# arobertlin/MinPaxos

Measured on AMD Instinct MI355X. Metric: decided+applied instances/sec (tally + KV apply + RCCL watermark all-reduce), higher is better.
Workload: dtype int32/int64

## Files before the change

### minpaxos_amd/csrc/step.hip

```cpp
#include "common.hpp"
#include "kernels.hpp"
#include "tally.hpp"

namespace mpx {

#ifndef MPX_STAMPS
#define MPX_STAMPS 0
#endif
#if MPX_STAMPS
__device__ unsigned long long mpx_stamp_acc[16];
constexpr uint32_t kSpanMax = 1u << 17;
__device__ unsigned long long mpx_wg_span[kSpanMax][2];
#define STAMP_DECL                                                     \
    unsigned long long _st_prev = 0, _st_rt0 = 0;                      \
    if (threadIdx.x == 0) {                                            \
        _st_prev = __builtin_amdgcn_s_memtime();                       \
        _st_rt0 = __builtin_amdgcn_s_memrealtime();                    \
    }
#define STAMP_SPAN()                                                   \
    do {                                                               \
        if (MPX_STAMPS >= 2 && threadIdx.x == 0 && blockIdx.x < kSpanMax) { \
            mpx_wg_span[blockIdx.x][0] = _st_rt0;                      \
            mpx_wg_span[blockIdx.x][1] = __builtin_amdgcn_s_memrealtime(); \
        }                                                              \
    } while (0)
#define STAMP(k)                                                       \
    do {                                                               \
        if (MPX_STAMPS == 1 && threadIdx.x == 0) {  \
            unsigned long long _n = __builtin_amdgcn_s_memtime();      \
            atomicAdd(&mpx_stamp_acc[k], _n - _st_prev);               \
            _st_prev = _n;                                             \
        }                                                              \
    } while (0)
#else
#define STAMP_DECL
#define STAMP(k)
#define STAMP_SPAN()
#endif
#ifndef MPX_ABLATE
#define MPX_ABLATE 0
#endif

#ifndef MPX_STEP_BALLOT
#define MPX_STEP_BALLOT 0
#endif

constexpr int kStepBlock = 256;
constexpr uint32_t kLock = 0xFFFFFFFFu;
constexpr uint32_t kDead = 0xFFFFFFFEu;
constexpr uint32_t kNoFirst = 0xFFFFFFFFu;

__device__ __forceinline__ uint32_t lhash(int64_t k) {
    uint64_t x = (uint64_t)k;
    x ^= x >> 33;
    x *= 0xff51afd7ed558ccdull;
    x ^= x >> 33;
    return (uint32_t)x;
}

struct Dict {
    int64_t* dkey;
    int64_t* dval;
    uint32_t* dfirst;
    uint32_t* cnt;
    uint32_t* hslot;
    uint8_t* dpresent;
    uint8_t* dseen;
    uint32_t* dn;
    uint32_t dcap, hcap;
};

__device__ int dict_insert(const Dict& D, int64_t key) {
    uint32_t h = lhash(key) & (D.hcap - 1);
    for (uint32_t probe = 0; probe < D.hcap;) {
        uint32_t cur = __hip_atomic_load(&D.hslot[h], __ATOMIC_ACQUIRE, __HIP_MEMORY_SCOPE_WORKGROUP);
        if (cur == 0) {
            const uint32_t old = atomicCAS(&D.hslot[h], 0u, kLock);
            if (old == 0) {
                const uint32_t kid = atomicAdd(D.dn, 1u);
                if (kid >= D.dcap) {
                    __hip_atomic_store(&D.hslot[h], kDead, __ATOMIC_RELEASE, __HIP_MEMORY_SCOPE_WORKGROUP);
                    return -1;
                }
                D.dkey[kid] = key;
                D.dval[kid] = 0;
                D.dpresent[kid] = 0;
                D.dseen[kid] = 0;
                D.dfirst[kid] = kNoFirst;
                D.cnt[kid] = 0;
                __hip_atomic_store(&D.hslot[h], kid + 1, __ATOMIC_RELEASE, __HIP_MEMORY_SCOPE_WORKGROUP);
                return (int)kid;
            }
            cur = old;
        }
        if (cur == kLock) continue;
        if (cur != kDead && D.dkey[cur - 1] == key) return (int)(cur - 1);
        h = (h + 1) & (D.hcap - 1);
        ++probe;
    }
    return -1;
}

__device__ __forceinline__ void dict_put_unique(const Dict& D, uint32_t e, int64_t k, int64_t v) {
    D.dkey[e] = k;
    D.dval[e] = v;
    D.dpresent[e] = 1;
    D.dseen[e] = 0;
    D.dfirst[e] = kNoFirst;
    uint32_t h = lhash(k) & (D.hcap - 1);
    while (atomicCAS(&D.hslot[h], 0u, e + 1) != 0u) h = (h + 1) & (D.hcap - 1);
}

template <int PER, typename OffT>
__device__ __forceinline__ void block_scan(const uint32_t* cnt, OffT* off, uint32_t n,
                                           uint32_t* wsum) {
    const int t = threadIdx.x, l = lane_id(), w = t / kWave;
    uint32_t v[PER];
    uint32_t sum = 0;
#pragma unroll
    for (int k = 0; k < PER; ++k) {
        const uint32_t i = t * PER + k;
        v[k] = i < n ? cnt[i] : 0;
        sum += v[k];
    }
    uint32_t incl = sum;
#pragma unroll
    for (int d = 1; d < kWave; d <<= 1) {
        const uint32_t x = __shfl_up(incl, d);
        if (l >= d) incl += x;
    }
    if (l == kWave - 1) wsum[w] = incl;
    __syncthreads();
    uint32_t wbase = 0;
    for (int k = 0; k < w; ++k) wbase += wsum[k];
    uint32_t run = wbase + incl - sum;
#pragma unroll
    for (int k = 0; k < PER; ++k) {
        const uint32_t i = t * PER + k;
        if (i < n) off[i] = (OffT)run;
        run += v[k];
    }
    __syncthreads();
}

template <typename OffT>
__device__ __forceinline__ uint8_t resolve_cmd(const Dict& D, const OffT* off,
                                               const uint16_t* list, const int64_t* cval, int kd,
                                               uint32_t li, uint8_t o, int64_t& r, bool& conf) {
    const bool isput = o == MPX_OP_PUT;
    int prev = -1, prevput = 0, lastput = -1;
    bool later = false, laterput = false;
    const uint32_t a = off[kd], z = a + D.cnt[kd];
    for (uint32_t j = a; j < z; ++j) {
        const uint32_t ent = list[j];
        const int lj = (int)(ent >> 1);
        const uint32_t pj = ent & 1u;
        if (lj < (int)li) {
            if (lj > prev) { prev = lj; prevput = (int)pj; }
            if (pj && lj > lastput) lastput = lj;
        } else if (lj > (int)li) {
            later = true;
            laterput |= pj != 0;
        }
    }
    const uint8_t seen = D.dseen[kd];
    if (prev >= 0) conf = prevput || isput;
    else conf = (seen & 1u) && ((seen & 2u) || isput);
    r = 0;
    if (isput) r = cval[li];
    else if (o == MPX_OP_GET) {
        if (lastput >= 0) r = cval[lastput];
        else if (D.dpresent[kd]) r = D.dval[kd];
    }
    uint8_t fl = 0;
    if (!later) fl |= 1;
    if (isput && !laterput) fl |= 2;
    if (isput && lastput < 0) fl |= 4;
    return fl;
}

__device__ __forceinline__ void apply_update(const Dict& D, int kd, uint8_t fl, uint8_t o,
                                             int64_t v, uint32_t first_pos, uint32_t n_orig) {
    if (fl & 1) D.dseen[kd] = (uint8_t)(1u | (o == MPX_OP_PUT ? 2u : 0u));
    if (fl & 2) {
        D.dval[kd] = v;
        D.dpresent[kd] = 1;
    }
    if ((fl & 4) && (uint32_t)kd >= n_orig && D.dfirst[kd] == kNoFirst) D.dfirst[kd] = first_pos;
}

__device__ __forceinline__ void table_writeback(const Dict& D, uint32_t norig, uint32_t dn,
                                                int64_t* kk, int64_t* kv, uint32_t kvpg,
                                                uint32_t* total, uint32_t* err) {
    const int t = threadIdx.x;
    for (uint32_t e = t; e < norig; e += kStepBlock) {
        kk[e] = D.dkey[e];
        kv[e] = D.dval[e];
    }
    if (t == 0) *total = norig;
    __syncthreads();
    for (uint32_t e = norig + t; e < dn; e += kStepBlock) {
        if (!D.dpresent[e]) continue;
        const uint32_t f = D.dfirst[e];
        uint32_t rank = 0;
        for (uint32_t x = norig; x < dn; ++x)
            if (D.dpresent[x] && D.dfirst[x] < f) ++rank;
        atomicAdd(total, 1u);
        const uint32_t dst = norig + rank;
        if (dst < kvpg) {
            kk[dst] = D.dkey[e];
            kv[dst] = D.dval[e];
        }
    }
    __syncthreads();
    if (t == 0 && *total > kvpg) raise_err(err, kErrKvFull);
}

template <int T_, int R_, int C_, int TB_, int HB_, int HN_ = (1 << HB_)>
struct FastCfg {
    static constexpr int kFT = T_, kFRecs = R_, kFIpg = T_, kFCmds = C_, kFTab = TB_;
    static constexpr int kFHB = HB_, kFH = HN_;
    static constexpr bool kFHPow2 = (HN_ & (HN_ - 1)) == 0;
    static_assert(HN_ <= (1 << HB_) && HN_ >= TB_ && HN_ % 8 == 0, "slot count");
    static constexpr int kFPer = kFCmds / kFT;
    static constexpr int kFRecPer = kFRecs / kFT;
    static constexpr int kFTabPer = (kFTab + kFT - 1) / kFT;
    static constexpr int kFWaves = kFT / kWave;
    static constexpr int kWaveCmds = kFCmds / kFWaves;
#ifndef MPX_DVAL_LDS_MAX
#define MPX_DVAL_LDS_MAX 512
#endif
    static constexpr bool kFDvalLds = TB_ <= MPX_DVAL_LDS_MAX;
    static_assert(kFCmds % kFT == 0 && kFRecs % kFT == 0, "whole items per thread");
    static_assert(kFCmds / 32 <= kWave, "the new-key bitmap is scanned by one wave");
    static_assert(kWaveCmds < 2047, "kTabLp holds 1 + a wave-relative command index");
    static_assert((kFH * 2) % 16 == 0, "the wave tables are cleared by 16-byte stores");
};
#ifndef MPX_FASTBASE_SLOTS
#define MPX_FASTBASE_SLOTS 512
#endif
using FastBase = FastCfg<256, 1024, 1024, 256, 9, MPX_FASTBASE_SLOTS>;
using FastRecs = FastCfg<256, 2048, 1024, 256, 9>;
using FastKeys = FastCfg<256, 1024, 1024, 1024, 10>;
using FastWide = FastCfg<512, 2048, 2048, 512, 10>;
using FastWide256 = FastCfg<512, 2048, 2048, 256, 9>;
constexpr uint16_t kNone16 = 0xFFFF;
constexpr uint8_t kIdBad = 31;
constexpr unsigned long long kFreeKey = 0x8000000000000000ull;
constexpr uint32_t kOverflow = 0x80000000u;
constexpr uint32_t kTabAny = 0x8000u;
constexpr uint32_t kTabPut = 0x4000u;
constexpr uint32_t kTabLp = 0x07FFu;

#define MPX_FAST_CONSTS                                                      \
    constexpr int kFT = Cfg::kFT, kFRecs = Cfg::kFRecs, kFIpg = Cfg::kFIpg;    \
    constexpr int kFCmds = Cfg::kFCmds, kFTab = Cfg::kFTab, kFH = Cfg::kFH;    \
    constexpr int kFPer = Cfg::kFPer, kFRecPer = Cfg::kFRecPer;                \
    constexpr int kFTabPer = Cfg::kFTabPer, kFWaves = Cfg::kFWaves;            \
    constexpr int kWaveCmds = Cfg::kWaveCmds;                                   \
    (void)kFT; (void)kFRecs; (void)kFIpg; (void)kFCmds; (void)kFTab; (void)kFH; \
    (void)kFPer; (void)kFRecPer; (void)kFTabPer; (void)kFWaves; (void)kWaveCmds;

template <class Cfg, int MODE>
struct FastLds {
    static constexpr int kFRecs = Cfg::kFRecs, kFIpg = Cfg::kFIpg, kFCmds = Cfg::kFCmds;
    static constexpr int kFTab = Cfg::kFTab, kFH = Cfg::kFH, kFWaves = Cfg::kFWaves;
    union {
        struct {
            int32_t inst[kFRecs];
            int32_t bal[MODE == MPX_MODE_CLASSIC ? kFRecs : 1];
            uint8_t idok[kFRecs];
            uint16_t rstart[kFIpg];
            uint16_t rend[kFIpg];
        } a;
        struct {
            int64_t cval[kFCmds];
            uint16_t tab[kFWaves * kFH];
#if !MPX_STEP_BALLOT
            uint8_t win[kFWaves * kFH];
            unsigned long long pmask[kFWaves * kWave];
#endif
        } b;
    } u;
    unsigned long long hkey[kFH];
    int64_t dval[Cfg::kFDvalLds ? kFTab : 1];
    uint16_t tabidx[kFH];
    uint32_t newbits[kFCmds / 32];
    uint16_t coff[kFIpg + 2];
    uint32_t red[1 + MPX_MAX_REPLICAS];
    uint32_t firstnil, firstbad, flags, ndec;
#ifdef MPX_LDS_PAD
    uint8_t lds_pad[MPX_LDS_PAD];
#endif
};

__device__ __forceinline__ uint32_t wave_max_u32(uint32_t v) {
#pragma unroll
    for (int d = 32; d >= 1; d >>= 1) {
        const uint32_t x = __shfl_xor(v, d);
        v = v > x ? v : x;
    }
    return (uint32_t)__builtin_amdgcn_readfirstlane((int)v);
}

template <int HB>
__device__ __forceinline__ uint32_t fhash(int64_t k) {
    const uint32_t x = (uint32_t)(uint64_t)k ^ (uint32_t)((uint64_t)k >> 32);
    return (x * 0x9E3779B1u) >> (32 - HB);
}
template <class Cfg>
__device__ __forceinline__ uint32_t fhome(int64_t k) {
    if constexpr (Cfg::kFHPow2) {
        return fhash<Cfg::kFHB>(k);
    } else {
        const uint32_t x = (uint32_t)(uint64_t)k ^ (uint32_t)((uint64_t)k >> 32);
        return (uint32_t)(((uint64_t)(x * 0x9E3779B1u) * (uint32_t)Cfg::kFH) >> 32);
    }
}

template <class Cfg, class Lds>
__device__ __forceinline__ int fast_slot(Lds& S, unsigned long long key, uint32_t h,
                                         int& fresh) {
    constexpr int kFH = Cfg::kFH;
    uint32_t i = h;
    for (int probe = 0; probe < kFH; ++probe) {
        const unsigned long long old = atomicCAS(&S.hkey[i], kFreeKey, key);
        if (old == kFreeKey || old == key) {
            fresh = old == kFreeKey;
            return (int)i;
        }
        i = Cfg::kFHPow2 ? (i + 1) & (kFH - 1) : (i + 1 == (uint32_t)kFH ? 0u : i + 1);
    }
    return -1;
}

constexpr uint32_t kPkGroups = 64;
__device__ __forceinline__ unsigned long long pk_word(uint32_t d, uint32_t xi, uint32_t xc) {
    return 1ull | ((unsigned long long)d << 7) | ((unsigned long long)xi << 23) |
           ((unsigned long long)xc << 39);
}
__device__ __forceinline__ uint32_t pk_slots(uint32_t n_groups) {
    return (n_groups + kPkGroups - 1) / kPkGroups;
}
__device__ void fold_packed(unsigned long long* pslots, uint32_t n_groups, int64_t* totals,
                            uint32_t* err) {
    __shared__ unsigned long long fsum[3];
    if (threadIdx.x < 3) fsum[threadIdx.x] = 0;
    __syncthreads();
    unsigned long long d = 0, xi = 0, xc = 0;
    const uint32_t nslots = pk_slots(n_groups);
    constexpr int kBatch = 2;
    for (uint32_t s0 = threadIdx.x; s0 < nslots; s0 += blockDim.x * kBatch) {
        unsigned long long w[kBatch];
#pragma unroll
        for (int k = 0; k < kBatch; ++k) {
            const uint32_t sl = s0 + k * blockDim.x;
            w[k] = sl < nslots ? __hip_atomic_load(pslots + sl, __ATOMIC_RELAXED,
                                                   __HIP_MEMORY_SCOPE_AGENT)
                               : 0ull;
        }
#pragma unroll
        for (int k = 0; k < kBatch; ++k) {
            const uint32_t sl = s0 + k * blockDim.x;
            if (sl >= nslots) continue;
            const uint32_t want = (n_groups - 1u - sl) / nslots + 1u;
            uint32_t spins = 0;
            bool late = false;
            while ((w[k] & 127ull) < want) {
                __builtin_amdgcn_s_sleep(2);
                w[k] = __hip_atomic_load(pslots + sl, __ATOMIC_RELAXED, __HIP_MEMORY_SCOPE_AGENT);
                if (++spins == (1u << 22)) {
                    raise_err(err, kErrInval | kErrSlots);
                    late = true;
                    break;
                }
            }
            if (!late) __hip_atomic_store(pslots + sl, 0ull, __ATOMIC_RELAXED, __HIP_MEMORY_SCOPE_AGENT);
            d += (w[k] >> 7) & 0xFFFFull;
            xi += (w[k] >> 23) & 0xFFFFull;
            xc += w[k] >> 39;
        }
    }
    if (d) atomicAdd(&fsum[0], d);
    if (xi) atomicAdd(&fsum[1], xi);
    if (xc) atomicAdd(&fsum[2], xc);
    __syncthreads();
    if (threadIdx.x < 3) totals[threadIdx.x] = (int64_t)fsum[threadIdx.x];
}

template <int MODE, class Cfg, bool kOne>
__global__ __launch_bounds__(Cfg::kFT) void k_group_fast(mpx_group_batch b, int32_t nrep,
                                                         uint32_t kvpg, uint32_t* worklist,
                                                         uint32_t* wcount,
                                                         unsigned long long* tacc, uint32_t* err,
                                                         unsigned long long* pslots,
                                                         int64_t* totals) {
    if constexpr (!kOne) {
        pslots = nullptr;
        totals = nullptr;
    }
    MPX_FAST_CONSTS
    __shared__ FastLds<Cfg, MODE> S;
    STAMP_DECL
    const uint32_t g = blockIdx.x;
    const int t = threadIdx.x, l = lane_id();
    const int32_t half = nrep >> 1;
    const uint32_t ipg = b.ipg;
    const uint64_t gi0 = (uint64_t)g * ipg;
    const uint64_t r0 = b.grp_rec_off[g], r1 = b.grp_rec_off[g + 1];
    const uint32_t c_lo = b.cmd_off[gi0], c_hi = b.cmd_off[gi0 + ipg];
    const uint32_t kcnt = b.kv_cnt_in[g];
    const int32_t cu_in = b.committed_in[g];
    const int32_t ex_in = b.executed_in[g];
    const uint64_t nrec = r1 - r0;
    const uint32_t ncmd = c_hi - c_lo;
    if (r1 < r0 || c_hi < c_lo || nrec > (uint64_t)kFRecs || ncmd > (uint32_t)kFCmds ||
        kcnt > (uint32_t)kFTab || kcnt > kvpg) {
        if (pslots) {
            if (t == 0) {
                raise_err(err, kErrInval);
                if (totals) (void)__hip_atomic_fetch_add(pslots + g % pk_slots(gridDim.x), 1ull, __ATOMIC_RELAXED,
                                                         __HIP_MEMORY_SCOPE_AGENT);
            }
            if (totals && g == gridDim.x - 1) fold_packed(pslots, gridDim.x, totals, err);
        } else if (t == 0) {
            worklist[atomicAdd(wcount, 1u)] = g;
        }
        return;
    }
    const int64_t lo = (int64_t)ex_in + 1 < 0 ? 0 : (int64_t)ex_in + 1;
    uint32_t ebits = 0;

    int4 rr[kFRecPer];
    if (nrec) {
        const uint32_t last = (uint32_t)nrec - 1;
#pragma unroll
        for (int k = 0; k < kFRecPer; ++k) {
            const uint32_t p = t + k * kFT;
            rr[k] = ld_stream(reinterpret_cast<const int4*>(b.recs) + r0 + (p < last ? p : last));
        }
    } else {
#pragma unroll
        for (int k = 0; k < kFRecPer; ++k) rr[k] = make_int4(-1, 0, 0, 0);
    }
    const bool own = (uint32_t)t < ipg;
    const uint32_t ti = own ? (uint32_t)t : ipg - 1;
    int4 st = ld_stream(reinterpret_cast<const int4*>(b.st_in) + gi0 + ti);
    const uint32_t co = b.cmd_off[gi0 + ti];
    const uint8_t hs = b.has_cmds ? b.has_cmds[gi0 + ti] : (uint8_t)1;
    int64_t tk[kFTabPer], tv[kFTabPer];
#pragma unroll
    for (int k = 0; k < kFTabPer; ++k) {
        const uint32_t e = (uint32_t)t + k * kFT;
        const uint64_t ei = (uint64_t)g * kvpg + (e < kcnt ? e : (kcnt ? kcnt - 1 : 0));
        tk[k] = b.kv_key_in[ei];
        tv[k] = b.kv_val_in[ei];
    }
#pragma unroll
    for (int k = 0; k < (kFH + kFT - 1) / kFT; ++k)
        if (kFH % kFT == 0 || t + k * kFT < kFH) S.hkey[t + k * kFT] = kFreeKey;
    for (int i = t; i < kFH / 2; i += kFT)
        reinterpret_cast<uint32_t*>(S.tabidx)[i] = 0xFFFFFFFFu;
    if (t < kFCmds / 32) S.newbits[t] = 0u;
    S.u.a.rstart[t] = kNone16;
    S.coff[t] = (uint16_t)(own ? co - c_lo : ncmd);
    if (t <= MPX_MAX_REPLICAS) S.red[t] = 0;
    if (t == 0) {
        S.coff[kFIpg] = (uint16_t)ncmd;
        S.firstnil = ipg;
        S.firstbad = ipg;
        S.flags = 0;
        S.ndec = 0;
    }
#pragma unroll
    for (int k = 0; k < kFRecPer; ++k) {
        const uint32_t p = t + k * kFT;
        const uint32_t idc = (rr[k].z >= 0 && rr[k].z < nrep) ? (uint32_t)rr[k].z : kIdBad;
        S.u.a.inst[p] = rr[k].x;
        if (MODE == MPX_MODE_CLASSIC) S.u.a.bal[p] = rr[k].y;
        S.u.a.idok[p] = (uint8_t)((idc << 1) | ((rr[k].w & 0xff) == 1 ? 1u : 0u));
    }
    const uint32_t clast = ncmd ? ncmd - 1 : 0;
    const uint32_t cbase = (uint32_t)(t - l) * kFPer + (uint32_t)l;
    uint8_t o[kFPer];
    int64_t ck[kFPer];
#pragma unroll
    for (int k = 0; k < kFPer; ++k) {
        const uint32_t li = cbase + k * kWave;
        const uint64_t ci = c_lo + (li < clast ? li : clast);
        o[k] = ncmd ? ld_stream(b.op + ci) : (uint8_t)0;
        ck[k] = ncmd ? ld_stream(b.key + ci) : 0;
    }
    __syncthreads();
    STAMP(0);

#pragma unroll
    for (int k = 0; k < kFRecPer; ++k) {
        const uint32_t p = t + k * kFT;
        const bool valid = p < nrec;
        const int32_t inst = S.u.a.inst[p];
        const int32_t prev = S.u.a.inst[p ? p - 1 : 0];
        const bool inwin = inst >= 0 && (uint32_t)inst < ipg;
        const bool pinwin = prev >= 0 && (uint32_t)prev < ipg;
        const bool head = valid && (p == 0 || inst != prev);
        ebits |= (valid && !inwin) ? kErrNil : 0u;
        ebits |= (head && p && inst < prev) ? kErrOrder : 0u;
        if (head && inwin) S.u.a.rstart[inst] = (uint16_t)p;
        if (head && p && pinwin) S.u.a.rend[prev] = (uint16_t)p;
        if (valid && p + 1 == nrec && inwin) S.u.a.rend[inst] = (uint16_t)nrec;
    }
    int tslot[kFTabPer];
#pragma unroll
    for (int k = 0; k < kFTabPer; ++k) {
        const uint32_t e = (uint32_t)t + k * kFT;
        tslot[k] = 0;
        if (e < kcnt) {
            int fresh = 0;
            const int sl = (unsigned long long)tk[k] == kFreeKey
                               ? -1
                               : fast_slot<Cfg>(S, (unsigned long long)tk[k], fhome<Cfg>(tk[k]),
                                           fresh);
            ebits |= sl < 0 ? kOverflow : 0u;
            tslot[k] = sl < 0 ? 0 : sl;
            if (fresh) S.tabidx[sl] = (uint16_t)e;
            if (Cfg::kFDvalLds) S.dval[e] = tv[k];
        }
    }
    __syncthreads();
    STAMP(1);

    bool dec = false;
#if MPX_ABLATE & 8
    const uint32_t ra = (uint32_t)t * 4;
    const bool touched = true;
    const uint32_t rn = 4;
#else
    const uint32_t ra = own ? S.u.a.rstart[t] : kNone16;
    const bool touched = ra != kNone16;
    const uint32_t rn = touched ? (uint32_t)S.u.a.rend[t] - ra : 0;
#endif
#if MPX_ABLATE & 1
    const uint32_t rmax = 0;
#else
    const uint32_t rmax = wave_max_u32(rn);
#endif
    if (MODE == MPX_MODE_MIN) {
        uint32_t idmask = 0;
        int32_t deci = 0;
        for (uint32_t j = 0; j < rmax; ++j) {
            const uint32_t p = j < rn ? ra + j : 0;
            const uint32_t io0 = S.u.a.idok[p];
            const uint32_t io = j < rn ? io0 : 0u;
            const int32_t okj = (int32_t)(io & 1u);
            const uint32_t nilbit = st.x == MPX_STATUS_NIL ? kErrNil : 0u;
            ebits |= okj ? nilbit : 0u;
            const int32_t oks = st.y + okj;
            const int32_t c1 = oks >= half ? okj : 0;
            const int32_t dj = oks == half ? c1 : 0;
            st.y = oks;
            st.x = dj ? MPX_COMMITTED : st.x;
            deci |= dj;
            const uint32_t id = io >> 1;
            const uint32_t badbit = id == kIdBad ? kErrBadId : 0u;
            ebits |= c1 ? badbit : 0u;
            idmask |= c1 ? (1u << id) : 0u;
        }
        dec = deci != 0;
        const uint32_t wbase = (uint32_t)(t - l) + 1;
        const unsigned long long dm = __ballot(deci != 0);
        if (l == 0 && dm) atomicMax(&S.red[0], wbase + 63u - (uint32_t)__clzll(dm));
        for (int i = 0; i < nrep; ++i) {
            const unsigned long long m = __ballot((idmask >> i) & 1u);
            if (l == 0 && m) atomicMax(&S.red[1 + i], wbase + 63u - (uint32_t)__clzll(m));
        }
    } else {
        ebits |= (touched && st.x == MPX_STATUS_NIL) ? kErrNil : 0u;
        int32_t deci = 0;
        for (uint32_t j = 0; j < rmax; ++j) {
            const uint32_t p = j < rn ? ra + j : 0;
            const int32_t act = j < rn ? 1 : 0;
            const int32_t io = (int32_t)S.u.a.idok[p];
            const int32_t bj = S.u.a.bal[p];
            const int32_t live = (uint32_t)(st.x - MPX_PREPARED) < 2u ? act : 0;
            const int32_t okj = live & io & 1;
            const int32_t nk = live & ((io & 1) ^ 1);
            const int32_t oks = st.y + okj;
            const int32_t c = oks >= half ? okj : 0;
            st.y = oks;
            st.x = c ? MPX_COMMITTED : st.x;
            deci |= c;
            st.z += nk;
            const int32_t nb = nk ? bj : INT32_MIN;
            st.w = st.w > nb ? st.w : nb;
        }
        dec = deci != 0;
        if (__ballot(dec) && l == 0) atomicMax(&S.red[0], 1u);
    }
    {
        const unsigned long long dm = __ballot(dec);
        if (l == 0 && dm) atomicAdd(&S.ndec, (uint32_t)__popcll(dm));
    }
    {
        uint32_t fn = (own && (int64_t)t >= lo && (st.x == MPX_STATUS_NIL || !hs)) ? (uint32_t)t : ipg;
        uint32_t fb = (MODE == MPX_MODE_CLASSIC && own && (int64_t)t >= (int64_t)cu_in + 1 &&
                       st.x != MPX_COMMITTED) ? (uint32_t)t : ipg;
#pragma unroll
        for (int d = 32; d >= 1; d >>= 1) {
            const uint32_t x = __shfl_xor(fn, d), y = __shfl_xor(fb, d);
            fn = fn < x ? fn : x;
            fb = fb < y ? fb : y;
        }
        if (l == 0) {
            if (fn < ipg) atomicMin(&S.firstnil, fn);
            if (MODE == MPX_MODE_CLASSIC && fb < ipg) atomicMin(&S.firstbad, fb);
        }
    }
    __syncthreads();
    STAMP(2);

    int32_t cu = cu_in;
    if (MPX_ABLATE & 32) {
        cu = (int32_t)ipg - 1;
    } else if (MODE == MPX_MODE_MIN) {
        if (S.red[0]) cu = (int32_t)S.red[0] - 1;
    } else if (S.red[0] && (int64_t)cu_in + 1 >= 0 && (int64_t)cu_in + 1 < (int64_t)ipg) {
        cu = (int32_t)S.firstbad - 1;
    }
    int64_t hi = (int64_t)cu;
    if (hi >= (int64_t)ipg) hi = (int64_t)ipg - 1;
    int64_t stop = hi >= lo ? hi + 1 : lo;
    if ((int64_t)S.firstnil < stop && (int64_t)S.firstnil >= lo) stop = S.firstnil;
    const uint32_t x0 = stop > lo ? S.coff[lo] : 0, x1 = stop > lo ? S.coff[stop] : 0;

    int64_t cv[kFPer];
#pragma unroll
    for (int k = 0; k < kFPer; ++k) {
        const uint32_t li = cbase + k * kWave;
        cv[k] = ncmd ? ld_stream(b.val + c_lo + (li < clast ? li : clast)) : 0;
    }
    uint32_t ops = 0;
#pragma unroll
    for (int k = 0; k < kFPer; ++k) ops |= (uint32_t)o[k] << (8 * k);
    const int wv = __builtin_amdgcn_readfirstlane(t / kWave);
    uint16_t* T = S.u.b.tab + wv * kFH;
#pragma unroll
    for (int k = 0; k < (kFH * 2 / 16 + kWave - 1) / kWave; ++k)
        if ((kFH * 2 / 16) % kWave == 0 || l + k * kWave < kFH * 2 / 16)
            reinterpret_cast<uint4*>(T)[l + k * kWave] = make_uint4(0u, 0u, 0u, 0u);
#if !MPX_STEP_BALLOT
    typedef __attribute__((address_space(3))) volatile uint8_t lds_u8;
    typedef __attribute__((address_space(3))) volatile unsigned long long lds_u64;
    lds_u8* W = (lds_u8*)(S.u.b.win + wv * kFH);
    lds_u64* PM = (lds_u64*)(S.u.b.pmask + wv * kWave);
    PM[l] = 0ull;
#endif
    const unsigned long long lanebit = 1ull << l;
    const unsigned long long below = lanebit - 1ull;
    const uint32_t wfirst = (uint32_t)wv * kWaveCmds;
    int kid[kFPer];
    uint32_t seen[kFPer];
#pragma unroll
    for (int k = 0; k < kFPer; ++k) {
        const uint32_t li = cbase + k * kWave;
        const bool act = li >= x0 && li < x1;
        const unsigned long long key = (unsigned long long)ck[k];
        int kd = -1;
#if MPX_ABLATE & 2
        if (act) kd = (int)fhome<Cfg>(ck[k]);
#else
        if (act && key != kFreeKey) {
            int fresh = 0;
            kd = fast_slot<Cfg>(S, key, fhome<Cfg>(ck[k]), fresh);
        }
#endif
        ebits |= (act && kd < 0) ? kOverflow : 0u;
        const bool live = act && kd >= 0;
        kid[k] = live ? kd : -1;
        const uint32_t sl = live ? (uint32_t)kd : 0u;
        const bool isput = ((ops >> (8 * k)) & 0xffu) == MPX_OP_PUT;
        const unsigned long long livem = __ballot(live);
        if (!livem) {
            seen[k] = 0;
            continue;
        }
        unsigned long long peers = 0;
#if MPX_STEP_BALLOT
        {
            unsigned long long m = livem;
#pragma unroll
            for (int i = 0; i < Cfg::kFHB; ++i) {
                const bool bit = (sl >> i) & 1u;
                const unsigned long long bm = __ballot(bit);
                m &= bit ? bm : ~bm;
            }
            peers = live ? m : 0ull;
        }
#else
        if (live) {
            W[sl] = (uint8_t)l;
            const uint32_t cls = W[sl];
            __hip_atomic_fetch_or((__attribute__((address_space(3))) unsigned long long*)&PM[cls],
                                  lanebit, __ATOMIC_RELAXED, __HIP_MEMORY_SCOPE_WORKGROUP);
            peers = PM[cls];
            PM[cls] = 0ull;
        }
#endif
        const unsigned long long putm = __ballot(live && isput);
        const unsigned long long lp_m = peers & below;
        const unsigned long long lput_m = lp_m & putm;
        const uint32_t e = live ? (uint32_t)T[sl] : 0u;
        const uint32_t rl1 = li - (uint32_t)l + 1u - wfirst;
        const uint32_t elp = e & kTabLp;
        const uint32_t hp = 63u - (uint32_t)__clzll(lp_m | 1ull);
        const uint32_t pflags = lp_m ? (kTabAny | (((putm >> hp) & 1ull) ? kTabPut : 0u))
                                     : (e & (kTabAny | kTabPut));
        const uint32_t lpr = lput_m ? rl1 + 63u - (uint32_t)__clzll(lput_m) : elp;
        seen[k] = pflags | (lpr ? lpr + wfirst : 0u);
        if (live && (peers >> l) == 1ull) {
            const unsigned long long allput = peers & putm;
            const uint32_t gl = allput ? rl1 + 63u - (uint32_t)__clzll(allput) : elp;
            T[sl] = (uint16_t)(kTabAny | (isput ? kTabPut : 0u) | gl);
        }
    }
#pragma unroll
    for (int k = 0; k < kFPer; ++k) S.u.b.cval[cbase + k * kWave] = cv[k];
    if (ebits & kOverflow) atomicOr(&S.flags, 1u);
    __syncthreads();
    STAMP(3);
    if (S.flags & 1u) {
        if (pslots) {
            if (t == 0) {
                raise_err(err, kErrInval);
                if (totals) (void)__hip_atomic_fetch_add(pslots + g % pk_slots(gridDim.x), 1ull, __ATOMIC_RELAXED,
                                                         __HIP_MEMORY_SCOPE_AGENT);
            }
            if (totals && g == gridDim.x - 1) fold_packed(pslots, gridDim.x, totals, err);
        } else if (t == 0) {
            worklist[atomicAdd(wcount, 1u)] = g;
        }
        return;
    }
    if (own) {
        if (!(MPX_ABLATE & 16) && touched) st_stream(reinterpret_cast<int4*>(b.st_out) + gi0 + t, st);
        if (b.decided) b.decided[gi0 + t] = dec ? 1 : 0;
    }
    STAMP(4);

    uint32_t fnew = 0;
#pragma unroll
    for (int k = 0; k < kFPer; ++k) {
        const uint32_t li = cbase + k * kWave;
        const bool act = kid[k] >= 0;
        if (!__ballot(act)) continue;
        const uint32_t sl = act ? (uint32_t)kid[k] : 0u;
        uint32_t pf = seen[k] & (kTabAny | kTabPut), lp = seen[k] & kTabLp;
        for (int w2 = wv - 1; w2 >= 0; --w2) {
            const uint32_t e = S.u.b.tab[w2 * kFH + sl];
            const uint32_t elp = e & kTabLp;
            pf = pf ? pf : (e & (kTabAny | kTabPut));
            lp = lp ? lp : (elp ? elp + (uint32_t)w2 * kWaveCmds : 0u);
        }
        const bool hasprev = pf != 0;
        const int lastput = (int)lp - 1;
        const uint32_t op = (ops >> (8 * k)) & 0xffu;
        const bool isput = op == MPX_OP_PUT;
        const bool prevput = (pf & kTabPut) != 0;
        const int src = isput ? (int)li : lastput;
        const int64_t sv = S.u.b.cval[src >= 0 ? src : 0];
        const uint32_t ti = S.tabidx[sl];
        const bool intab = ti != kNone16;
        const int64_t at_start =
            Cfg::kFDvalLds ? S.dval[intab ? ti : 0]
                           : (intab && op == MPX_OP_GET && lastput < 0
                                  ? b.kv_val_in[(uint64_t)g * kvpg + ti]
                                  : 0);
        const int64_t r = isput ? sv : (op == MPX_OP_GET ? (lastput >= 0 ? sv : (intab ? at_start : 0)) : 0);
        const bool conf = hasprev && (prevput || isput);
        if (act) {
            st_stream(b.ret + c_lo + li, r);
            if (b.conf_prev) st_stream(b.conf_prev + c_lo + li, (uint8_t)(conf ? 1 : 0));
            if (isput && lastput < 0 && !intab) {
                fnew |= 1u << k;
                atomicOr(&S.newbits[li >> 5], 1u << (li & 31));
            }
        }
    }
    __syncthreads();
    STAMP(5);

    auto last_put = [&](uint32_t sl) {
        uint32_t m = 0;
#pragma unroll
        for (int w2 = 0; w2 < kFWaves; ++w2) {
            const uint32_t x = S.u.b.tab[w2 * kFH + sl] & kTabLp;
            m = x ? x + (uint32_t)w2 * kWaveCmds : m;
        }
        return m;
    };
    int64_t* kko = b.kv_key_out + (uint64_t)g * kvpg;
    int64_t* kvo = b.kv_val_out + (uint64_t)g * kvpg;
#pragma unroll
    for (int k = 0; k < kFTabPer; ++k) {
        const uint32_t e = (uint32_t)t + k * kFT;
        if (!(MPX_ABLATE & 16) && e < kcnt) {
            const uint32_t dl = last_put((uint32_t)tslot[k]);
            kko[e] = (int64_t)S.hkey[tslot[k]];
            kvo[e] = dl ? S.u.b.cval[dl - 1] : (Cfg::kFDvalLds ? S.dval[e] : tv[k]);
        }
    }
    const uint32_t wbits = l < kFCmds / 32 ? S.newbits[l] : 0u;
    const uint32_t pc = __popc(wbits);
    uint32_t incl = pc;
#pragma unroll
    for (int d = 1; d < kFCmds / 32; d <<= 1) {
        const uint32_t x = __shfl_up(incl, d);
        if (l >= d) incl += x;
    }
    const uint32_t excl = incl - pc;
    const uint32_t n_new = (uint32_t)__shfl((int)incl, kFCmds / 32 - 1);
    const uint32_t total = kcnt + n_new;
#pragma unroll
    for (int k = 0; k < kFPer; ++k) {
        const uint32_t li = cbase + k * kWave;
        const uint32_t base = (uint32_t)__shfl((int)excl, (int)(li >> 5));
        const uint32_t rank = base + __popc(S.newbits[li >> 5] & ((1u << (li & 31)) - 1u));
        if (!(MPX_ABLATE & 16) && ((fnew >> k) & 1u) && kcnt + rank < kvpg) {
            const uint32_t kd = (uint32_t)kid[k];
            kko[kcnt + rank] = (int64_t)S.hkey[kd];
            kvo[kcnt + rank] = S.u.b.cval[last_put(kd) - 1];
        }
    }
    ebits |= (t == 0 && total > kvpg) ? kErrKvFull : 0u;
    if (t < nrep) {
        const uint32_t k = MODE == MPX_MODE_MIN ? S.red[1 + t] : 0u;
        b.peer_out[(uint64_t)g * nrep + t] =
            k ? (int32_t)k - 2 : b.peer_in[(uint64_t)g * nrep + t];
    }
    if (t == 0) {
        b.committed_out[g] = cu;
        b.executed_out[g] = stop > lo ? (int32_t)(stop - 1) : ex_in;
        b.kv_cnt_out[g] = total < kvpg ? total : kvpg;
        if (b.n_decided) b.n_decided[g] = S.ndec;
    }
    if (tacc && t < 3) {
        const uint32_t v = t == 0 ? S.ndec : (stop > lo ? (t == 1 ? (uint32_t)(stop - lo) : x1 - x0) : 0u);
        if (v)
            (void)__hip_atomic_fetch_add(tacc + (g & (kTotSlots - 1)) * 3 + t, (unsigned long long)v,
                                         __ATOMIC_RELAXED, __HIP_MEMORY_SCOPE_AGENT);
    }
    if (pslots && totals && t == 0)
        (void)__hip_atomic_fetch_add(pslots + g % pk_slots(gridDim.x),
                                     pk_word(S.ndec, stop > lo ? (uint32_t)(stop - lo) : 0u,
                                             stop > lo ? x1 - x0 : 0u),
                                     __ATOMIC_RELAXED, __HIP_MEMORY_SCOPE_AGENT);
    ebits &= 0x7FFFFFFFu;
    if (ebits) raise_err(err, ebits);
    if (pslots && totals && g == gridDim.x - 1) fold_packed(pslots, gridDim.x, totals, err);
    STAMP(6);
    STAMP_SPAN();
}

constexpr int kDCap = 2048;
constexpr int kHCap = 2 * kDCap;
constexpr int kChunk = 1024;
constexpr int kPer = kChunk / kStepBlock;
constexpr int kMaxIpgBits = 8192;

struct GenLds {
    int64_t dkey[kDCap];
    int64_t dval[kDCap];
    uint32_t dfirst[kDCap];
    uint32_t cnt[kDCap];
    uint32_t off[kDCap];
    uint32_t hslot[kHCap];
    int64_t cval[kChunk];
    uint16_t list[kChunk];
    uint8_t dpresent[kDCap];
    uint8_t dseen[kDCap];
    uint32_t dec_bits[kMaxIpgBits / 32];
    uint32_t wsum[kStepBlock / kWave];
    unsigned long long red[1 + MPX_MAX_REPLICAS];
    uint32_t dn, n_orig, ndec, scal[4];
};

template <int MODE>
__device__ void group_general(GenLds& S, const mpx_group_batch& b, uint32_t g, int32_t nrep,
                             uint32_t kvpg, unsigned long long* tacc, uint32_t* err) {
    const int t = threadIdx.x, l = lane_id(), w = t / kWave;
    const int32_t half = nrep >> 1;
    const uint64_t ipg = b.ipg;
    const uint64_t gi0 = (uint64_t)g * ipg;
    const mpx_inst_state* st_in = b.st_in + gi0;
    mpx_inst_state* st_out = b.st_out + gi0;

    if (t <= MPX_MAX_REPLICAS) S.red[t] = 0;
    for (int i = t; i < kMaxIpgBits / 32; i += kStepBlock) S.dec_bits[i] = 0;
    for (int i = t; i < kHCap; i += kStepBlock) S.hslot[i] = 0;
    if (t == 0) {
        S.dn = 0;
        S.ndec = 0;
    }
    __syncthreads();

    const uint64_t r0 = b.grp_rec_off[g], r1 = b.grp_rec_off[g + 1];
    if (r1 > r0) {
        const uint64_t len = r1 - r0;
        const uint64_t n0 = r0 + len * w / (kStepBlock / kWave);
        const uint64_t n1 = r0 + len * (w + 1) / (kStepBlock / kWave);
        const uint64_t s = find_head(b.recs, n0, r0, r1);
        const uint64_t e = (n1 >= r1) ? r1 : find_head(b.recs, n1, r0, r1);
        if (s < e) {
            TallyOut out{0, 0, false};
            tally_range<MODE>(b.recs, s, e, st_in, st_out, ipg, 0, half, nrep, nullptr, err, 0,
                              out, S.dec_bits);
            if (MODE == MPX_MODE_MIN) {
                if (l == 0 && out.cu_key) atomicMax(&S.red[0], (unsigned long long)out.cu_key);
                if (l < nrep && out.pc_key) atomicMax(&S.red[1 + l], (unsigned long long)out.pc_key);
            } else {
                if (l == 0 && out.any_dec) atomicMax(&S.red[0], 1ull);
            }
        }
    } else if (r1 < r0) {
        raise_err(err, kErrInval);
    }
    __syncthreads();
    if (b.decided)
        for (uint64_t i = t; i < ipg; i += kStepBlock)
            b.decided[gi0 + i] = (S.dec_bits[i >> 5] >> (i & 31)) & 1u;
    if (b.n_decided) {
        uint32_t c = 0;
        for (uint64_t i = t; i < (ipg + 31) / 32; i += kStepBlock) c += __popc(S.dec_bits[i]);
        if (c) atomicAdd(&S.ndec, c);
    }

    const int32_t cu_in = b.committed_in[g];
    int32_t cu = cu_in;
    if (MPX_ABLATE & 32) {
        cu = (int32_t)ipg - 1;
    } else if (MODE == MPX_MODE_MIN) {
        if (S.red[0]) cu = (int32_t)(uint32_t)(S.red[0] & 0xffffffffull);
        if (t < nrep) {
            const unsigned long long k = S.red[1 + t];
            b.peer_out[(uint64_t)g * nrep + t] =
                k ? (int32_t)(uint32_t)(k & 0xffffffffull) : b.peer_in[(uint64_t)g * nrep + t];
        }
    } else {
        if (t < nrep) b.peer_out[(uint64_t)g * nrep + t] = b.peer_in[(uint64_t)g * nrep + t];
        if (S.red[0]) {
            if (t == 0) S.scal[1] = (uint32_t)ipg;
            __syncthreads();
            const int64_t j0 = (int64_t)cu_in + 1;
            if (j0 >= 0 && (uint64_t)j0 < ipg) {
                for (uint64_t j = (uint64_t)j0 + t; j < ipg; j += kStepBlock) {
                    const bool dec = (S.dec_bits[j >> 5] >> (j & 31)) & 1u;
                    if (!(dec || st_in[j].status == MPX_COMMITTED)) {
                        atomicMin(&S.scal[1], (uint32_t)j);
                        break;
                    }
                }
            }
            __syncthreads();
            if (j0 >= 0 && (uint64_t)j0 < ipg) cu = (int32_t)S.scal[1] - 1;
        }
    }
    if (t == 0) b.committed_out[g] = cu;

    const int32_t ex_in = b.executed_in[g];
    int64_t lo = (int64_t)ex_in + 1;
    int64_t hi = (int64_t)cu;
    if (hi >= (int64_t)ipg) hi = (int64_t)ipg - 1;
    if (lo < 0) lo = 0;
    if (t == 0) S.scal[2] = (uint32_t)(hi + 1 > lo ? hi + 1 : lo);
    __syncthreads();
    if (hi >= lo) {
        for (int64_t i = lo + t; i <= hi; i += kStepBlock) {
            const bool nil = st_in[i].status == MPX_STATUS_NIL || (b.has_cmds && !b.has_cmds[gi0 + i]);
            if (nil) {
                atomicMin(&S.scal[2], (uint32_t)i);
                break;
            }
        }
    }
    __syncthreads();
    const int64_t stop = hi >= lo ? (int64_t)S.scal[2] : lo;
    if (t == 0) {
        b.executed_out[g] = stop > lo ? (int32_t)(stop - 1) : ex_in;
        if (b.n_decided) b.n_decided[g] = S.ndec;
    }
    if (tacc && t == 0) {
        unsigned long long* p = tacc + (g & (kTotSlots - 1)) * 3;
        if (S.ndec) atomic_add_done(p, (unsigned long long)S.ndec);
        if (stop > lo) {
            atomic_add_done(p + 1, (unsigned long long)(stop - lo));
            const uint64_t xc = b.cmd_off[gi0 + stop] - b.cmd_off[gi0 + lo];
            if (xc) atomic_add_done(p + 2, (unsigned long long)xc);
        }
    }

    const Dict D{S.dkey, S.dval, S.dfirst, S.cnt, S.hslot, S.dpresent, S.dseen, &S.dn,
                 (uint32_t)kDCap, (uint32_t)kHCap};
    const uint32_t ncnt = b.kv_cnt_in[g];
    if (ncnt > kvpg || ncnt > (uint32_t)kDCap) {
        raise_err(err, kErrInval);
        return;
    }
    for (uint32_t e = t; e < ncnt; e += kStepBlock)
        dict_put_unique(D, e, b.kv_key_in[(uint64_t)g * kvpg + e], b.kv_val_in[(uint64_t)g * kvpg + e]);
    if (t == 0) {
        S.dn = ncnt;
        S.n_orig = ncnt;
    }
    __syncthreads();

    if (stop > lo) {
        const uint64_t c_begin = b.cmd_off[gi0 + lo], c_end = b.cmd_off[gi0 + stop];
        for (uint64_t c0 = c_begin; c0 < c_end; c0 += kChunk) {
            const uint32_t n = (uint32_t)((c_end - c0) < (uint64_t)kChunk ? (c_end - c0) : kChunk);
            for (uint32_t i = t; i < (uint32_t)kDCap; i += kStepBlock) S.cnt[i] = 0;
            __syncthreads();
            uint8_t o[kPer];
            int kid[kPer];
            uint32_t pos[kPer];
#pragma unroll
            for (int k = 0; k < kPer; ++k) {
                const uint32_t li = t + k * kStepBlock;
                kid[k] = -1;
                o[k] = 0;
                if (li < n) {
                    o[k] = b.op[c0 + li];
                    S.cval[li] = b.val[c0 + li];
                    kid[k] = dict_insert(D, b.key[c0 + li]);
                    if (kid[k] >= 0) pos[k] = atomicAdd(&S.cnt[kid[k]], 1u);
                    else raise_err(err, kErrKvFull);
                }
            }
            __syncthreads();
            const uint32_t dn = S.dn < (uint32_t)kDCap ? S.dn : (uint32_t)kDCap;
            block_scan<kDCap / kStepBlock>(S.cnt, S.off, dn, S.wsum);
#pragma unroll
            for (int k = 0; k < kPer; ++k) {
                const uint32_t li = t + k * kStepBlock;
                if (li < n && kid[k] >= 0)
                    S.list[S.off[kid[k]] + pos[k]] = (uint16_t)((li << 1) | (o[k] == MPX_OP_PUT ? 1u : 0u));
            }
            __syncthreads();
            uint8_t fl[kPer];
#pragma unroll
            for (int k = 0; k < kPer; ++k) {
                const uint32_t li = t + k * kStepBlock;
                fl[k] = 0;
                if (li >= n || kid[k] < 0) continue;
                int64_t r;
                bool conf;
                fl[k] = resolve_cmd(D, S.off, S.list, S.cval, kid[k], li, o[k], r, conf);
                b.ret[c0 + li] = r;
                if (b.conf_prev) b.conf_prev[c0 + li] = conf ? 1 : 0;
            }
            __syncthreads();
#pragma unroll
            for (int k = 0; k < kPer; ++k) {
                const uint32_t li = t + k * kStepBlock;
                if (li < n && kid[k] >= 0)
                    apply_update(D, kid[k], fl[k], o[k], S.cval[li], (uint32_t)(c0 + li - c_begin),
                                 S.n_orig);
            }
            __syncthreads();
        }
    }
    const uint32_t dn = S.dn < (uint32_t)kDCap ? S.dn : (uint32_t)kDCap;
    table_writeback(D, S.n_orig, dn, b.kv_key_out + (uint64_t)g * kvpg,
                    b.kv_val_out + (uint64_t)g * kvpg, kvpg, &S.scal[0], err);
    if (t == 0) b.kv_cnt_out[g] = S.scal[0] < kvpg ? S.scal[0] : kvpg;
}

__device__ __forceinline__ void group_totals(const mpx_group_batch& b, uint32_t g,
                                             unsigned long long& d, unsigned long long& xi,
                                             unsigned long long& xc) {
    d = b.n_decided[g];
    const int64_t ei = b.executed_in[g], eo = b.executed_out[g];
    const int64_t lo = ei + 1 < 0 ? 0 : ei + 1;
    xi = xc = 0;
    if (eo >= lo && eo < (int64_t)b.ipg) {
        const uint64_t gi0 = (uint64_t)g * b.ipg;
        xi = (unsigned long long)(eo - lo + 1);
        xc = b.cmd_off[gi0 + eo + 1] - b.cmd_off[gi0 + lo];
    }
}

template <int MODE>
__global__ __launch_bounds__(kStepBlock) void k_group_general(mpx_group_batch b, int32_t nrep,
                                                              uint32_t kvpg,
                                                              const uint32_t* worklist,
                                                              uint32_t* wcount,
                                                              int64_t* totals, uint32_t* err) {
    __shared__ GenLds S;
    __shared__ bool last;
    __shared__ unsigned long long fold[3];
    unsigned long long* part = reinterpret_cast<unsigned long long*>(wcount + 16);
    auto fold_totals = [&]() {
        if (threadIdx.x < 3) fold[threadIdx.x] = 0;
        __syncthreads();
        if (threadIdx.x < kTotSlots * 3) {
            const unsigned long long v = atomic_take(part + threadIdx.x);
            if (v) atomicAdd(&fold[threadIdx.x % 3], v);
        }
        __syncthreads();
        if (threadIdx.x < 3) totals[threadIdx.x] = (int64_t)fold[threadIdx.x];
    };
    static_assert(kTotSlots * 3 <= kStepBlock, "one partial slot word per thread");
    const uint32_t n = *wcount;
    if (n == 0) {
        if (totals && blockIdx.x == 0) fold_totals();
        return;
    }
    const uint32_t workers = n < gridDim.x ? n : gridDim.x;
    if (blockIdx.x >= workers) return;
    for (uint32_t i = blockIdx.x; i < n; i += gridDim.x) {
        group_general<MODE>(S, b, worklist[i], nrep, kvpg, totals ? part : nullptr, err);
        __syncthreads();
    }
    __syncthreads();
    if (threadIdx.x == 0) {
        const uint32_t k = __hip_atomic_fetch_add(wcount + 1, 1u, __ATOMIC_RELAXED,
                                                  __HIP_MEMORY_SCOPE_AGENT);
        last = k == workers - 1;
        if (last) {
            wcount[0] = 0;
            wcount[1] = 0;
        }
    }
    __syncthreads();
    if (last && totals) fold_totals();
}

__global__ void k_fill_worklist(uint32_t* worklist, uint32_t* wcount, uint32_t n) {
    const uint32_t i = blockIdx.x * blockDim.x + threadIdx.x;
    if (i < n) worklist[i] = i;
    if (i == 0) *wcount = n;
}

namespace {
void record_timing_event(hipEvent_t ev, hipStream_t stream) {
    hipStreamCaptureStatus cs = hipStreamCaptureStatusNone;
    (void)hipStreamIsCapturing(stream, &cs);
    if (cs == hipStreamCaptureStatusActive)
        (void)hipEventRecordWithFlags(ev, stream, hipEventRecordExternal);
    else
        (void)hipEventRecord(ev, stream);
}

template <int MODE, class Cfg>
void launch_fast(const mpx_group_batch* b, int32_t nrep, uint32_t kvpg, uint32_t* worklist,
                 uint32_t* wcount, unsigned long long* tacc, uint32_t* err, hipStream_t stream,
                 unsigned long long* pslots, int64_t* totals) {
    if (pslots)
        k_group_fast<MODE, Cfg, true><<<b->n_groups, Cfg::kFT, 0, stream>>>(
            *b, nrep, kvpg, worklist, wcount, tacc, err, pslots, totals);
    else
        k_group_fast<MODE, Cfg, false><<<b->n_groups, Cfg::kFT, 0, stream>>>(
            *b, nrep, kvpg, worklist, wcount, tacc, err, nullptr, nullptr);
}
int fast_variant(int32_t nrep, uint32_t ipg, uint32_t kvpg) {
    const uint64_t recs = (uint64_t)(nrep > 1 ? nrep - 1 : 1) * ipg;
    if (ipg <= 256 && recs <= 1024 && kvpg <= 256) return 1;
    if (ipg <= 256 && recs <= 2048 && kvpg <= 256) return 2;
    if (ipg <= 256 && recs <= 1024 && kvpg <= 1024) return 3;
    if (ipg <= 512 && recs <= 2048 && kvpg <= 256) return 5;
    if (ipg <= 512 && recs <= 2048 && kvpg <= 512) return 4;
    return 0;
}
template <int MODE>
void launch_step(const mpx_group_batch* b, int32_t nrep, uint32_t kvpg, uint32_t* worklist,
                 uint32_t* wcount, int64_t* totals, uint32_t* err, hipStream_t stream,
                 hipEvent_t ev0, hipEvent_t ev1, unsigned long long* pslots) {
    unsigned long long* const tacc =
        totals && !pslots ? reinterpret_cast<unsigned long long*>(wcount + 16) : nullptr;
    int64_t* const ptot = pslots ? totals : nullptr;
    if (ev0) record_timing_event(ev0, stream);
    switch (fast_variant(nrep, b->ipg, kvpg)) {
#define MPX_FAST_CASE(n, C)                                                                    \
    case n:                                                                                    \
        launch_fast<MODE, C>(b, nrep, kvpg, worklist, wcount, tacc, err, stream, pslots, ptot); \
        break;
    MPX_FAST_CASE(1, FastBase)
    MPX_FAST_CASE(2, FastRecs)
    MPX_FAST_CASE(3, FastKeys)
    MPX_FAST_CASE(4, FastWide)
    MPX_FAST_CASE(5, FastWide256)
#undef MPX_FAST_CASE
    default:
        k_fill_worklist<<<(b->n_groups + 255) / 256, 256, 0, stream>>>(worklist, wcount,
                                                                       b->n_groups);
    }
    if (ev1) record_timing_event(ev1, stream);
    if (pslots) return;
    const unsigned gen_grid = b->n_groups < 256 ? b->n_groups : 256;
    k_group_general<MODE><<<gen_grid ? gen_grid : 1, kStepBlock, 0, stream>>>(
        *b, nrep, kvpg, worklist, wcount, totals, err);
}
}

bool step_one_launch_fits(int32_t nrep, uint32_t ipg, uint32_t kv_per_group) {
    return fast_variant(nrep, ipg, kv_per_group) != 0;
}

hipError_t launch_group_step(int mode, int32_t nrep, uint32_t kv_per_group,
                             const mpx_group_batch* b, uint32_t* worklist, uint32_t* wcount,
                             int64_t* totals, uint32_t* err, hipStream_t stream,
                             hipEvent_t ev0, hipEvent_t ev1, unsigned long long* pslots) {
    if (!b->n_groups)
        return totals ? hipMemsetAsync(totals, 0, 3 * sizeof(int64_t), stream) : hipSuccess;
    if (kv_per_group > (uint32_t)kDCap) return hipErrorInvalidValue;
    if (b->ipg > (uint32_t)kMaxIpgBits) return hipErrorInvalidValue;
    if (pslots && !step_one_launch_fits(nrep, b->ipg, kv_per_group)) return hipErrorInvalidValue;
    if (mode == MPX_MODE_MIN)
        launch_step<MPX_MODE_MIN>(b, nrep, kv_per_group, worklist, wcount, totals, err, stream,
                                  ev0, ev1, pslots);
    else
        launch_step<MPX_MODE_CLASSIC>(b, nrep, kv_per_group, worklist, wcount, totals, err,
                                      stream, ev0, ev1, pslots);
    return hipGetLastError();
}

__global__ __launch_bounds__(256) void k_step_totals(mpx_group_batch b, unsigned long long* totals,
                                                     uint32_t* ctl) {
    unsigned long long* acc = reinterpret_cast<unsigned long long*>(ctl + 4);
    __shared__ unsigned long long red[3][kStepBlock / kWave];
    const uint32_t g = blockIdx.x * blockDim.x + threadIdx.x;
    unsigned long long d = 0, xi = 0, xc = 0;
    if (g < b.n_groups) group_totals(b, g, d, xi, xc);
#pragma unroll
    for (int k = 32; k >= 1; k >>= 1) {
        d += __shfl_xor(d, k);
        xi += __shfl_xor(xi, k);
        xc += __shfl_xor(xc, k);
    }
    const int w = threadIdx.x / kWave;
    if (lane_id() == 0) {
        red[0][w] = d;
        red[1][w] = xi;
        red[2][w] = xc;
    }
    __syncthreads();
    if (threadIdx.x < 3) {
        unsigned long long v = 0;
        for (int k = 0; k < kStepBlock / kWave; ++k) v += red[threadIdx.x][k];
        if (v) atomic_add_done(acc + threadIdx.x, v);
    }
    if (last_workgroup(ctl + 10) && threadIdx.x < 3)
        totals[threadIdx.x] = atomic_take(acc + threadIdx.x);
}

hipError_t launch_step_totals(const mpx_group_batch* b, int64_t* totals, uint32_t* ctl,
                              hipStream_t stream) {
    const uint32_t blocks = b->n_groups ? (b->n_groups + kStepBlock - 1) / kStepBlock : 1;
    k_step_totals<<<blocks, kStepBlock, 0, stream>>>(*b, reinterpret_cast<unsigned long long*>(totals),
                                                     ctl);
    return hipGetLastError();
}

}

#if MPX_STAMPS
extern "C" int mpx_debug_stamps(unsigned long long* out16, int reset) {
    if (hipMemcpyFromSymbol(out16, HIP_SYMBOL(mpx::mpx_stamp_acc), 16 * sizeof(unsigned long long)) != hipSuccess)
        return -3;
    if (reset) {
        unsigned long long z[16] = {0};
        if (hipMemcpyToSymbol(HIP_SYMBOL(mpx::mpx_stamp_acc), z, sizeof(z)) != hipSuccess) return -3;
    }
    return 0;
}
extern "C" int mpx_debug_spans(unsigned long long* out, unsigned n) {
    if (n > mpx::kSpanMax) n = mpx::kSpanMax;
    return hipMemcpyFromSymbol(out, HIP_SYMBOL(mpx::mpx_wg_span), (size_t)n * 16) == hipSuccess ? 0 : -3;
}
#endif
```

Baseline: 23.16 billion.

## Alias chunk-match scratch into cval slice, raise occupancy hint, batch table lookups

The per-wave window bytes and peer masks used for chunk matching now live inside that wave's own slice of the cval array instead of separate LDS arrays. This shrinks the shared-memory footprint so more workgroups can be resident. The FastBase config also passes a minimum-waves-per-SIMD hint of 8 to launch_bounds for the non-kOne kernel, which caps register use. The post-tally lookup loop is split into phases so all table, cval and tabidx loads for a thread's commands are issued together before any results are computed. The risks are register spills under the tighter bound and correctness hazards from aliasing scratch with cval, which a compiler memory barrier is added to guard.

```diff
diff --git a/minpaxos_amd/csrc/step.hip b/minpaxos_amd/csrc/step.hip
--- a/minpaxos_amd/csrc/step.hip
+++ b/minpaxos_amd/csrc/step.hip
@@ -216,7 +216,7 @@
     if (t == 0 && *total > kvpg) raise_err(err, kErrKvFull);
 }
 
-template <int T_, int R_, int C_, int TB_, int HB_, int HN_ = (1 << HB_)>
+template <int T_, int R_, int C_, int TB_, int HB_, int HN_ = (1 << HB_), int WPS_ = 1>
 struct FastCfg {
     static constexpr int kFT = T_, kFRecs = R_, kFIpg = T_, kFCmds = C_, kFTab = TB_;
     static constexpr int kFHB = HB_, kFH = HN_;
@@ -226,6 +226,7 @@
     static constexpr int kFRecPer = kFRecs / kFT;
     static constexpr int kFTabPer = (kFTab + kFT - 1) / kFT;
     static constexpr int kFWaves = kFT / kWave;
+    static constexpr int kFMinWavesPerSimd = WPS_;
     static constexpr int kWaveCmds = kFCmds / kFWaves;
 #ifndef MPX_DVAL_LDS_MAX
 #define MPX_DVAL_LDS_MAX 512
@@ -235,11 +236,16 @@
     static_assert(kFCmds / 32 <= kWave, "the new-key bitmap is scanned by one wave");
     static_assert(kWaveCmds < 2047, "kTabLp holds 1 + a wave-relative command index");
     static_assert((kFH * 2) % 16 == 0, "the wave tables are cleared by 16-byte stores");
+    static constexpr int kScratchWin = 0, kScratchMask = kFH;
+    static_assert(kWaveCmds * 8 >= kFH + kWave * 8, "the chunk-match scratch fits the wave's cval slice");
+    static_assert(kWaveCmds == kFPer * kWave && kWaveCmds * kFWaves == kFCmds,
+                  "a wave's commands are one contiguous slice of cval: the slice is wave-private");
+    static_assert(kScratchMask % 8 == 0, "the masks are 8-byte aligned");
 };
 #ifndef MPX_FASTBASE_SLOTS
 #define MPX_FASTBASE_SLOTS 512
 #endif
-using FastBase = FastCfg<256, 1024, 1024, 256, 9, MPX_FASTBASE_SLOTS>;
+using FastBase = FastCfg<256, 1024, 1024, 256, 9, MPX_FASTBASE_SLOTS, 8>;
 using FastRecs = FastCfg<256, 2048, 1024, 256, 9>;
 using FastKeys = FastCfg<256, 1024, 1024, 1024, 10>;
 using FastWide = FastCfg<512, 2048, 2048, 512, 10>;
@@ -276,10 +282,6 @@
         struct {
             int64_t cval[kFCmds];
             uint16_t tab[kFWaves * kFH];
-#if !MPX_STEP_BALLOT
-            uint8_t win[kFWaves * kFH];
-            unsigned long long pmask[kFWaves * kWave];
-#endif
         } b;
     } u;
     unsigned long long hkey[kFH];
@@ -389,8 +391,8 @@
 }
 
 template <int MODE, class Cfg, bool kOne>
-__global__ __launch_bounds__(Cfg::kFT) void k_group_fast(mpx_group_batch b, int32_t nrep,
-                                                         uint32_t kvpg, uint32_t* worklist,
+__global__ __launch_bounds__(Cfg::kFT, kOne ? 1 : Cfg::kFMinWavesPerSimd)
+void k_group_fast(mpx_group_batch b, int32_t nrep, uint32_t kvpg, uint32_t* worklist,
                                                          uint32_t* wcount,
                                                          unsigned long long* tacc, uint32_t* err,
                                                          unsigned long long* pslots,
@@ -650,8 +652,9 @@
 #if !MPX_STEP_BALLOT
     typedef __attribute__((address_space(3))) volatile uint8_t lds_u8;
     typedef __attribute__((address_space(3))) volatile unsigned long long lds_u64;
-    lds_u8* W = (lds_u8*)(S.u.b.win + wv * kFH);
-    lds_u64* PM = (lds_u64*)(S.u.b.pmask + wv * kWave);
+    uint8_t* const slice = reinterpret_cast<uint8_t*>(S.u.b.cval + wv * kWaveCmds);
+    lds_u8* W = (lds_u8*)(slice + Cfg::kScratchWin);
+    lds_u64* PM = (lds_u64*)(slice + Cfg::kScratchMask);
     PM[l] = 0ull;
 #endif
     const unsigned long long lanebit = 1ull << l;
@@ -722,6 +725,9 @@
             T[sl] = (uint16_t)(kTabAny | (isput ? kTabPut : 0u) | gl);
         }
     }
+#if !MPX_STEP_BALLOT
+    __asm__ volatile("" ::: "memory");
+#endif
 #pragma unroll
     for (int k = 0; k < kFPer; ++k) S.u.b.cval[cbase + k * kWave] = cv[k];
     if (ebits & kOverflow) atomicOr(&S.flags, 1u);
@@ -747,43 +753,68 @@
     STAMP(4);
 
     uint32_t fnew = 0;
-#pragma unroll
-    for (int k = 0; k < kFPer; ++k) {
-        const uint32_t li = cbase + k * kWave;
-        const bool act = kid[k] >= 0;
-        if (!__ballot(act)) continue;
-        const uint32_t sl = act ? (uint32_t)kid[k] : 0u;
-        uint32_t pf = seen[k] & (kTabAny | kTabPut), lp = seen[k] & kTabLp;
+    {
+        uint32_t sl[kFPer], pf[kFPer], lp[kFPer];
+#pragma unroll
+        for (int k = 0; k < kFPer; ++k) {
+            sl[k] = kid[k] >= 0 ? (uint32_t)kid[k] : 0u;
+            pf[k] = seen[k] & (kTabAny | kTabPut);
+            lp[k] = seen[k] & kTabLp;
+        }
         for (int w2 = wv - 1; w2 >= 0; --w2) {
-            const uint32_t e = S.u.b.tab[w2 * kFH + sl];
-            const uint32_t elp = e & kTabLp;
-            pf = pf ? pf : (e & (kTabAny | kTabPut));
-            lp = lp ? lp : (elp ? elp + (uint32_t)w2 * kWaveCmds : 0u);
-        }
-        const bool hasprev = pf != 0;
-        const int lastput = (int)lp - 1;
-        const uint32_t op = (ops >> (8 * k)) & 0xffu;
-        const bool isput = op == MPX_OP_PUT;
-        const bool prevput = (pf & kTabPut) != 0;
-        const int src = isput ? (int)li : lastput;
-        const int64_t sv = S.u.b.cval[src >= 0 ? src : 0];
-        const uint32_t ti = S.tabidx[sl];
-        const bool intab = ti != kNone16;
-        const int64_t at_start =
-            Cfg::kFDvalLds ? S.dval[intab ? ti : 0]
-                           : (intab && op == MPX_OP_GET && lastput < 0
-                                  ? b.kv_val_in[(uint64_t)g * kvpg + ti]
-                                  : 0);
-        const int64_t r = isput ? sv : (op == MPX_OP_GET ? (lastput >= 0 ? sv : (intab ? at_start : 0)) : 0);
-        const bool conf = hasprev && (prevput || isput);
-        if (act) {
-            st_stream(b.ret + c_lo + li, r);
-            if (b.conf_prev) st_stream(b.conf_prev + c_lo + li, (uint8_t)(conf ? 1 : 0));
-            if (isput && lastput < 0 && !intab) {
-                fnew |= 1u << k;
+            uint32_t e[kFPer];
+#pragma unroll
+            for (int k = 0; k < kFPer; ++k) e[k] = S.u.b.tab[w2 * kFH + sl[k]];
+#pragma unroll
+            for (int k = 0; k < kFPer; ++k) {
+                const uint32_t elp = e[k] & kTabLp;
+                pf[k] = pf[k] ? pf[k] : (e[k] & (kTabAny | kTabPut));
+                lp[k] = lp[k] ? lp[k] : (elp ? elp + (uint32_t)w2 * kWaveCmds : 0u);
+            }
+        }
+        int64_t sv[kFPer], at_start[kFPer];
+        uint32_t ti[kFPer];
+#pragma unroll
+        for (int k = 0; k < kFPer; ++k) {
+            const uint32_t li = cbase + k * kWave;
+            const bool isput = ((ops >> (8 * k)) & 0xffu) == MPX_OP_PUT;
+            const int src = isput ? (int)li : (int)lp[k] - 1;
+            sv[k] = S.u.b.cval[src >= 0 ? src : 0];
+            ti[k] = S.tabidx[sl[k]];
+        }
+#pragma unroll
+        for (int k = 0; k < kFPer; ++k) {
+            const uint32_t op = (ops >> (8 * k)) & 0xffu;
+            const bool intab = ti[k] != kNone16;
+            at_start[k] = Cfg::kFDvalLds ? S.dval[intab ? ti[k] : 0]
+                                         : (kid[k] >= 0 && intab && op == MPX_OP_GET && lp[k] == 0
+                                                ? b.kv_val_in[(uint64_t)g * kvpg + ti[k]]
+                                                : 0);
+        }
+#pragma unroll
+        for (int k = 0; k < kFPer; ++k) {
+            const uint32_t li = cbase + k * kWave;
+            const bool act = kid[k] >= 0;
+            const bool hasprev = pf[k] != 0;
+            const int lastput = (int)lp[k] - 1;
+            const uint32_t op = (ops >> (8 * k)) & 0xffu;
+            const bool isput = op == MPX_OP_PUT;
+            const bool prevput = (pf[k] & kTabPut) != 0;
+            const bool intab = ti[k] != kNone16;
+            const int64_t r = isput ? sv[k] : (op == MPX_OP_GET ? (lastput >= 0 ? sv[k] : (intab ? at_start[k] : 0)) : 0);
+            const bool conf = hasprev && (prevput || isput);
+            if (act) {
+                st_stream(b.ret + c_lo + li, r);
+                if (b.conf_prev) st_stream(b.conf_prev + c_lo + li, (uint8_t)(conf ? 1 : 0));
+                if (isput && lastput < 0 && !intab) fnew |= 1u << k;
+            }
+        }
+#pragma unroll
+        for (int k = 0; k < kFPer; ++k)
+            if ((fnew >> k) & 1u) {
+                const uint32_t li = cbase + k * kWave;
                 atomicOr(&S.newbits[li >> 5], 1u << (li & 31));
             }
-        }
     }
     __syncthreads();
     STAMP(5);
```

After: 22.34 billion. 0.965x the previous value.
